# magic-research/vector_quantization

Hardware: AMD Instinct MI355X
Metric: quantized tokens/sec, VQGAN quantizer forward K=16384 D=256 (higher is better)
Workload: dtype f16+f32; 1 GPU; VQGAN K=16384 D=256, 256x256 images -> 16x16 tokens, bf16 latents, VQGANQuantizer.forward of the drop-in nn.Module, eval mode (prepare+argmin+gather+STE+loss); images_per_gpu=2048, parallelism=dp1 (independent shards, no data-path collective)

## Files before the change

vector_quantization_amd/csrc/vqhip.hip:

```cpp
#include "vqhip.h"

#include <hip/hip_runtime.h>
#include <stdio.h>
#include <string.h>

#include "vqhip_kernels.h"
#include "vqhip_fsq_kernels.h"

static thread_local char g_err[256] = "";

static int fail(int code, const char *what, const char *detail = "") {
    snprintf(g_err, sizeof(g_err), "%s%s%s", what, detail[0] ? ": " : "", detail);
    return code;
}

#define VQ_CHECK_LAUNCH(name)                                            \
    do {                                                                 \
        hipError_t err__ = hipGetLastError();                            \
        if (err__ != hipSuccess) return fail(VQHIP_ELAUNCH, name, hipGetErrorString(err__)); \
    } while (0)

#define VQ_HIP(call)                                                     \
    do {                                                                 \
        hipError_t err__ = (call);                                       \
        if (err__ != hipSuccess) return fail(VQHIP_ELAUNCH, #call, hipGetErrorString(err__)); \
    } while (0)

#include <atomic>
#include <mutex>
#include <vector>
static std::atomic<bool> g_prof_on{false};
static std::mutex g_prof_mu;
static std::vector<std::pair<hipEvent_t, hipEvent_t>> g_prof_events;
static size_t g_prof_used = 0;

static long prof_begin(hipStream_t s) {
    if (!g_prof_on.load(std::memory_order_relaxed)) return -1;
    std::lock_guard<std::mutex> lock(g_prof_mu);
    if (g_prof_used == g_prof_events.size()) {
        hipEvent_t a, b;
        if (hipEventCreate(&a) != hipSuccess || hipEventCreate(&b) != hipSuccess) { g_prof_on = false; return -1; }
        g_prof_events.emplace_back(a, b);
    }
    const long slot = (long)g_prof_used++;
    (void)hipEventRecord(g_prof_events[slot].first, s);
    return slot;
}
static void prof_end(long slot, hipStream_t s) {
    if (slot < 0) return;
    std::lock_guard<std::mutex> lock(g_prof_mu);
    if ((size_t)slot < g_prof_events.size()) (void)hipEventRecord(g_prof_events[slot].second, s);
}

#define VQ_MAX_DEVICES 64
typedef std::atomic<size_t> LdsCache[VQ_MAX_DEVICES];
static int ensure_dyn_lds(const void *kern, size_t bytes, LdsCache &set) {
    int dev = 0;
    VQ_HIP(hipGetDevice(&dev));
    const bool cached = dev >= 0 && dev < VQ_MAX_DEVICES;
    if (!cached || bytes > set[dev].load(std::memory_order_acquire)) {
        VQ_HIP(hipFuncSetAttribute(kern, hipFuncAttributeMaxDynamicSharedMemorySize, (int)bytes));
        if (cached) {
            size_t cur = set[dev].load(std::memory_order_relaxed);
            while (cur < bytes && !set[dev].compare_exchange_weak(cur, bytes, std::memory_order_release)) {}
        }
    }
    return VQHIP_OK;
}

#define VQ_NEED(what, have, need)                                                                         \
    do {                                                                                                  \
        const int64_t need__ = (need);                                                                    \
        if ((have) < need__) {                                                                            \
            char msg__[160];                                                                              \
            snprintf(msg__, sizeof(msg__), "%lld bytes given, %lld needed", (long long)(have), (long long)need__); \
            return fail(VQHIP_EINVAL, what, msg__);                                                       \
        }                                                                                                 \
    } while (0)

static inline int waves_grid(int64_t rows, int waves_per_block) {
    return (int)((rows + waves_per_block - 1) / waves_per_block);
}

static std::atomic<int> g_tune_slices{0};
static std::atomic<int> g_tune_force_exact{0};
static std::atomic<int> g_tune_stream{1};
#define VQ_FUSED_DECIDE_MAX_N 16384

template <int NSTEP, int TT, int WAVES, int TPS, int NBUF = 2, bool FILTER = false, bool NOAUX = false, bool GROUPS = false, int XD = 0>
static int launch_coarse_cfg(const char *ximg, int64_t N, const char *frag, int64_t nstages, int nslices, float *rec,
                             int64_t Np, const VqCbStats *cbst, const float *xh2, const float *rho2, int Dp, int metric,
                             const VqDecideOut &dec, int pad_stage, int tpb, hipStream_t s) {
    constexpr int LDS = NBUF * (TPS * NSTEP + VQ_AUX_CHUNKS(TPS)) * VQ_CHUNK_BYTES;
    auto kern = coarse_kernel<NSTEP, TT, WAVES, TPS, NBUF, FILTER, NOAUX, GROUPS, XD>;
    static LdsCache lds_set;
    if (int rc = ensure_dyn_lds((const void *)kern, LDS, lds_set)) return rc;
    const int64_t ntiles = (N + 15) / 16;
    const int64_t ntb = (ntiles + tpb - 1) / tpb;
    const int grid = (int)(ntb * nslices);
    const long slot = prof_begin(s);
    kern<<<grid, WAVES * 64, LDS, s>>>(ximg, N, frag, nstages, nslices, rec, Np, cbst, xh2, rho2, Dp, metric, dec, pad_stage, tpb);
    prof_end(slot, s);
    VQ_CHECK_LAUNCH("coarse_kernel");
    return VQHIP_OK;
}

template <int TT, int WAVES, int TPS, int NBUF, bool NOAUX, int KS>
static int launch_coarse32_cfg(const char *ximg, int64_t N, const char *frag, int64_t nstages, int nslices, float *rec,
                               int64_t Np, const VqCbStats *cbst, const float *xh2, const float *rho2, int Dp, int metric,
                               const int *n_dev, const VqGroupLists &grp, int pad_stage, int tpb, hipStream_t s) {
    constexpr int LDS = NBUF * (TPS * 2 + VQ_AUX_CHUNKS(TPS)) * VQ_CHUNK_BYTES;
    auto kern = coarse32_kernel<TT, WAVES, TPS, NBUF, NOAUX, KS, VQ_GROUP_TILES>;
    static LdsCache lds_set;
    if (int rc = ensure_dyn_lds((const void *)kern, LDS, lds_set)) return rc;
    const int64_t ntiles = (N + 15) / 16;
    const int64_t ntb = (ntiles + tpb - 1) / tpb;
    const long slot = prof_begin(s);
    kern<<<(int)(ntb * nslices), WAVES * 64, LDS, s>>>(ximg, N, frag, nstages, nslices, rec, Np, cbst, xh2, rho2, Dp, metric, n_dev, grp, pad_stage, tpb);
    prof_end(slot, s);
    VQ_CHECK_LAUNCH("coarse32_kernel");
    return VQHIP_OK;
}

template <int NSTEP, int TT, int WAVES, int TPS, int NBUF = 2, int XD = 0>
static int launch_rescan_cfg(const char *ximg, const char *frag, int64_t nstages, const int *rescan_list, const int *counters,
                             const float *thr, int *rescan_cnt, int *cand_list, hipStream_t s, const void *xrows = nullptr) {
    constexpr int LDS = NBUF * (TPS * NSTEP + VQ_AUX_CHUNKS(TPS)) * VQ_CHUNK_BYTES + WAVES * TT * 16 * 4 * (1 + VQ_RESCAN_LOCAL);
    auto kern = rescan_kernel<NSTEP, TT, WAVES, TPS, NBUF, XD>;
    static LdsCache lds_set;
    if (int rc = ensure_dyn_lds((const void *)kern, LDS, lds_set)) return rc;
    kern<<<256, WAVES * 64, LDS, s>>>(ximg, frag, nstages, rescan_list, counters, thr, rescan_cnt, cand_list, xrows);
    VQ_CHECK_LAUNCH("rescan_kernel");
    return VQHIP_OK;
}

#ifndef VQ_W32_MAX_D
#define VQ_W32_MAX_D 32
#endif
#ifndef VQ_NBUF_D32
#define VQ_NBUF_D32 4
#endif
#ifndef VQ_D32_SMALL_TT
#define VQ_D32_SMALL_TT 2
#define VQ_D32_SMALL_W 8
#endif
#ifndef VQ_MIN_SLICES_FILTER
#define VQ_MIN_SLICES_FILTER 1
#endif
static int balanced_tiles_per_block(int64_t N, int full) {
    if (full < 16) return full;
    const int64_t ntiles = (N + 15) / 16;
    int best = full;
    int64_t best_cost = ((ntiles + full - 1) / full + 255) / 256 * full;
    for (int tpb = full - 1; tpb >= full / 2 && tpb >= 8; --tpb) {
        const int64_t cost = ((ntiles + tpb - 1) / tpb + 255) / 256 * tpb;
        if (cost < best_cost) { best_cost = cost; best = tpb; }
    }
    return best;
}

static bool vq_xdirect(int64_t N, int64_t K, int D, int x_dtype, int metric, const int *n_dev) {
    if (D != 256 || n_dev != nullptr || vq_cb_layout(K, D).nstages < 2 || g_tune_slices.load() == 1) return false;
    if (x_dtype != VQHIP_DTYPE_BF16) return false;
    if (metric != VQHIP_METRIC_L2 && metric != VQHIP_METRIC_COS && metric != VQHIP_METRIC_COS_BF16) return false;
    if (N <= VQ_FUSED_DECIDE_MAX_N) return false;
    return !(N <= 4096 || (N <= 256 * 64 && K <= 4096));
}

static int pick_slices(int64_t ntb, int64_t nstages, int min_slices = 2) {
    if (const int forced = g_tune_slices.load(); forced > 0) { int ns = forced; while (ns > 1 && ns > nstages) ns >>= 1; return ns; }
    int64_t want = (256 + ntb - 1) / ntb;
    want = want < min_slices ? min_slices : want;
    int ns = 1;
    while (ns < want && ns < VQ_MAX_SLICES) ns <<= 1;
    while (ns > 1 && ns > nstages) ns >>= 1;
    return ns;
}

struct VqGroupRun { int used, ks, noaux, pad_stage; };
static int launch_coarse(const char *ximg, int64_t N, const VqCbLayout &L, const char *frag, float *rec, int64_t Np,
                         const VqCbStats *cbst, const float *xh2, const float *rho2, int metric, const VqDecideOut &dec,
                         int *nslices_out, int *fused_decide_out, hipStream_t s, VqGroupLists grp = VqGroupLists{nullptr, nullptr, nullptr, nullptr, 0, 1, 0},
                         VqGroupRun *grun = nullptr, bool xd = false) {
    const int nstep = L.nstep;
    const bool small = N <= 256 * 64;
    const bool small16 = N <= 4096 || (N <= 256 * 64 && L.K <= 4096);
    const bool small32 = N < 512 * 512;
    const bool noaux = !VQ_IS_L2(metric);
    const int pad_stage = (L.K % ((int64_t)L.tps * VQ_TILE_CODES)) ? (int)(L.nstages - 1) : -1;
#define VQ_CFG(NS, TT, W, ...)                                                                      \
    {                                                                                               \
        int64_t ntb = (N + (W) * (TT) * 16 - 1) / ((W) * (TT) * 16);                                \
        int ns = pick_slices(ntb, L.nstages, (NS) <= 8 ? VQ_MIN_SLICES_FILTER : 2);                 \
        *nslices_out = ns;                                                                          \
        const int tpb = (ns == 1) ? balanced_tiles_per_block(N, (W) * (TT)) : (W) * (TT);           \
        VqDecideOut dsel = dec;                                                                     \
        if (!(ns == 1 || N <= VQ_FUSED_DECIDE_MAX_N)) dsel.idx = nullptr;                           \
        *fused_decide_out = dsel.idx != nullptr ? 1 : 0;                                            \
        return launch_coarse_cfg<NS, TT, W, __VA_ARGS__>(ximg, N, frag, L.nstages, ns, rec, Np, cbst, xh2, rho2, L.Dp, metric, dsel, pad_stage, tpb, s); \
    }
    switch (nstep) {
        case 2: if ((L.D <= 16 || (L.D <= VQ_W32_MAX_D && noaux)) && N >= VQ_W32_MIN_N && grp.bcnt != nullptr && grun != nullptr) {
                    const int tt = small32 ? 1 : 2;
                    const int full = 8 * tt * 2;
                    const int64_t ntb0 = (N + full * 16 - 1) / (full * 16);
                    int ns = pick_slices(ntb0, L.nstages, VQ_MIN_SLICES_FILTER);
                    ns = ns > VQ_GROUP_MAX_SLICES ? VQ_GROUP_MAX_SLICES : ns;
                    *nslices_out = ns;
                    int tpb = (ns == 1) ? balanced_tiles_per_block(N, full) : full;
                    tpb = (tpb + 1) & ~1;
                    *fused_decide_out = 0;
                    grun->used = 1; grun->ks = L.D <= 16 ? 1 : 2; grun->noaux = noaux ? 1 : 0; grun->pad_stage = pad_stage;
#define VQ_CFG32(TTW, NOAUXV, KSV) return launch_coarse32_cfg<TTW, 8, VQ_TPS_D32, VQ_NBUF_D32, NOAUXV, KSV>(ximg, N, frag, L.nstages, ns, rec, Np, cbst, xh2, rho2, L.Dp, metric, dec.n_dev, grp, pad_stage, tpb, s)
                    if (L.D <= 16) {
                        if (tt == 1) { if (noaux) VQ_CFG32(1, true, 1); else VQ_CFG32(1, false, 1); }
                        else { if (noaux) VQ_CFG32(2, true, 1); else VQ_CFG32(2, false, 1); }
                    } else {
                        if (tt == 1) { if (noaux) VQ_CFG32(1, true, 2); else VQ_CFG32(1, false, 2); }
                        else { if (noaux) VQ_CFG32(2, true, 2); else VQ_CFG32(2, false, 2); }
                    }
#undef VQ_CFG32
                }
                if (N >= VQ_GROUPS_MIN_N) {
                    if (noaux) { if (small32) VQ_CFG(2, VQ_D32_SMALL_TT, VQ_D32_SMALL_W, VQ_TPS_D32, VQ_NBUF_D32, true, true, true) else VQ_CFG(2, 4, 8, VQ_TPS_D32, VQ_NBUF_D32, true, true, true) }
                    if (small32) VQ_CFG(2, VQ_D32_SMALL_TT, VQ_D32_SMALL_W, VQ_TPS_D32, VQ_NBUF_D32, true, false, true) else VQ_CFG(2, 4, 8, VQ_TPS_D32, VQ_NBUF_D32, true, false, true)
                }
                if (noaux) { if (small32) VQ_CFG(2, VQ_D32_SMALL_TT, VQ_D32_SMALL_W, VQ_TPS_D32, VQ_NBUF_D32, true, true) else VQ_CFG(2, 4, 8, VQ_TPS_D32, VQ_NBUF_D32, true, true) }
                if (small32) VQ_CFG(2, VQ_D32_SMALL_TT, VQ_D32_SMALL_W, VQ_TPS_D32, VQ_NBUF_D32, true) else VQ_CFG(2, 4, 8, VQ_TPS_D32, VQ_NBUF_D32, true)
        case 4: if (small) VQ_CFG(4, 2, 8, 4, 4, true) else VQ_CFG(4, 4, 8, 4, 4, true)
        case 8: if (small) VQ_CFG(8, 2, 8, 4, 4, true) else VQ_CFG(8, 4, 8, 4, 4, true)
        case 16: if (xd && !small16) VQ_CFG(16, 4, 8, VQ_TPS16, 4, false, false, false, 1)
                 if (small16) VQ_CFG(16, 2, 8, VQ_TPS16, 4) else VQ_CFG(16, 4, 8, VQ_TPS16, 4)
        case 32: VQ_CFG(32, 2, 8, 2)
        case 48: VQ_CFG(48, 2, 8, 1)
        case 64: {
            auto cost = [&](int tokens, double eff) {
                const int64_t ntb = (N + tokens - 1) / tokens;
                const int ns = pick_slices(ntb, L.nstages, 2);
                return (double)((ntb * ns + 255) / 256) * tokens * ((double)L.nstages / ns) / eff;
            };
            if (cost(192, 1.18) < cost(128, 1.0)) VQ_CFG(64, 3, 4, 1) else VQ_CFG(64, 1, 8, 1)
        }
        default: break;
    }
#undef VQ_CFG
    return fail(VQHIP_EINVAL, "vqhip_argmin: unsupported padded D");
}

static int resident_grid(int per_cu) {
    static std::atomic<int> cus[VQ_MAX_DEVICES];
    int dev = 0, n = 0;
    if (hipGetDevice(&dev) != hipSuccess) return 256 * per_cu;
    if (dev >= 0 && dev < VQ_MAX_DEVICES && (n = cus[dev].load(std::memory_order_relaxed)) > 0) return n * per_cu;
    if (hipDeviceGetAttribute(&n, hipDeviceAttributeMultiprocessorCount, dev) != hipSuccess || n <= 0) n = 256;
    if (dev >= 0 && dev < VQ_MAX_DEVICES) cus[dev].store(n, std::memory_order_relaxed);
    return n * per_cu;
}

template <int MODE>
static int run_exact_tiled(const void *x, int x_dtype, const float *e, const float *en, const float *xn, int64_t N, int64_t K,
                           int D, int metric, u64 *keys, float *dout, hipStream_t s) {
    const int bf = x_dtype == VQHIP_DTYPE_F32 ? 0 : 1;
    const int64_t items = ((N + 127) / 128) * ((K + 255) / 256);
    if (g_tune_stream.load() && D % (bf ? 8 : 4) == 0 && items < (int64_t)1 << 31) {
        static LdsCache ssets[2];
        const int lds = vq_xs_lds_bytes(bf);
        const void *kern = bf ? (const void *)exact_stream_kernel<1, MODE> : (const void *)exact_stream_kernel<0, MODE>;
        if (int rc = ensure_dyn_lds(kern, lds, ssets[bf])) return rc;
        const int cap = resident_grid(2);
        const int grid = (int)(items < cap ? items : cap);
        if (bf) exact_stream_kernel<1, MODE><<<grid, 256, lds, s>>>(x, e, en, xn, N, K, D, metric, keys, dout);
        else exact_stream_kernel<0, MODE><<<grid, 256, lds, s>>>(x, e, en, xn, N, K, D, metric, keys, dout);
        VQ_CHECK_LAUNCH("exact_stream_kernel");
        return VQHIP_OK;
    }
    constexpr int LDS = 2 * 32 * 128 * 4 + 8 * 32 * 4;
    static LdsCache sets[4];
    const void *kerns[4] = {(const void *)exact_tiled_kernel<0, MODE, false>, (const void *)exact_tiled_kernel<1, MODE, false>,
                            (const void *)exact_tiled_kernel<0, MODE, true>, (const void *)exact_tiled_kernel<1, MODE, true>};
    const int v4 = (D % 4 == 0) ? 2 : 0;
    if (int rc = ensure_dyn_lds(kerns[v4 + bf], LDS, sets[v4 + bf])) return rc;
    int grid = (int)(items < 1024 ? items : 1024);
#define VQ_TILED(DT, V4) exact_tiled_kernel<DT, MODE, V4><<<grid, 256, LDS, s>>>(x, e, en, xn, N, K, D, metric, keys, dout)
    if (v4) { if (bf) VQ_TILED(1, true); else VQ_TILED(0, true); }
    else { if (bf) VQ_TILED(1, false); else VQ_TILED(0, false); }
#undef VQ_TILED
    VQ_CHECK_LAUNCH("exact_tiled_kernel");
    return VQHIP_OK;
}

static int exact_few_max(int D) {
    if (D > 512 || D > VQ_FEW_MAX_D) return 0;
    static std::atomic<int> lds_limit{-1};
    int lim = lds_limit.load(std::memory_order_relaxed);
    if (lim < 0) {
        int dev = 0, v = 0;
        if (hipGetDevice(&dev) != hipSuccess || hipDeviceGetAttribute(&v, hipDeviceAttributeMaxSharedMemoryPerBlock, dev) != hipSuccess) v = 65536;
        lim = v;
        lds_limit.store(lim);
    }
    return vq_few_lds_bytes(D) <= lim ? VQ_EXACT_FEW_MAX : 0;
}

static int run_exact_rows(const void *x, int x_dtype, const float *e, const float *en, const float *xn, int64_t N, int64_t K, int D,
                          int metric, const int *row_list, const int *nrows_dev, u64 *keys, int *ticket, int64_t *idx,
                          int32_t *hist, hipStream_t s) {
    const int64_t ncb = (K + 63) / 64;
    const int grid = (int)(ncb < 256 ? 256 : (ncb > 1024 ? 1024 : ncb));
    if (D % 4) return fail(VQHIP_EINVAL, "exact_kernel: D % 4 != 0 (the proposal route has D % 8 == 0)");
    const int few_max = exact_few_max(D);
    const int lds = few_max ? vq_few_lds_bytes(D) : 0;
    static LdsCache sets[2];
    const int bf = x_dtype == VQHIP_DTYPE_F32 ? 0 : 1;
    if (int rc = ensure_dyn_lds(bf ? (const void *)exact_kernel<1> : (const void *)exact_kernel<0>, lds, sets[bf])) return rc;
    if (!bf)
        exact_kernel<0><<<grid, 256, lds, s>>>(x, e, en, xn, N, K, D, metric, row_list, nrows_dev, keys, ticket, idx, hist, few_max);
    else
        exact_kernel<1><<<grid, 256, lds, s>>>(x, e, en, xn, N, K, D, metric, row_list, nrows_dev, keys, ticket, idx, hist, few_max);
    VQ_CHECK_LAUNCH("exact_kernel");
    return VQHIP_OK;
}

template <int MODE>
static int run_segsum(const void *src, int x_dtype, const float *e, const int64_t *idx, const int32_t *order,
                      const int32_t *offsets, int64_t N, int64_t K, int D, const float *g_cb, float *dst, void *ws,
                      hipStream_t s) {
    float *partial = (float *)ws;
    const int64_t nranges = (N + VQ_SEG_RANGE - 1) / VQ_SEG_RANGE;
    int grid = (int)((nranges + 3) / 4); grid = grid < 1 ? 1 : (grid > 4096 ? 4096 : grid);
    if (x_dtype == VQHIP_DTYPE_F32) segsum_rows_kernel<MODE, 0><<<grid, 256, 0, s>>>(src, e, idx, order, offsets, N, (int)K, D, g_cb, dst, partial);
    else segsum_rows_kernel<MODE, 1><<<grid, 256, 0, s>>>(src, e, idx, order, offsets, N, (int)K, D, g_cb, dst, partial);
    VQ_CHECK_LAUNCH("segsum_rows_kernel");
    int fgrid = (int)((K + 3) / 4); fgrid = fgrid > 2048 ? 2048 : fgrid;
    segsum_fixup_kernel<<<fgrid, 256, 0, s>>>(offsets, (int)K, D, partial, dst);
    VQ_CHECK_LAUNCH("segsum_fixup_kernel");
    return VQHIP_OK;
}

template <bool NORMALIZE>
static int launch_row_small(const void *v, int dtype, int64_t R, int D, float eps, float *out, hipStream_t s) {
    const int L = D <= 8 ? 8 : (D <= 16 ? 16 : 32);
    const int grid = waves_grid((R + 64 / L - 1) / (64 / L), 4);
#define VQ_ROW_SMALL(DT, LL) row_small_kernel<DT, LL, NORMALIZE><<<grid, 256, 0, s>>>(v, R, D, eps, out)
    if (dtype == VQHIP_DTYPE_F32) { if (L == 8) VQ_ROW_SMALL(0, 8); else if (L == 16) VQ_ROW_SMALL(0, 16); else VQ_ROW_SMALL(0, 32); }
    else { if (L == 8) VQ_ROW_SMALL(1, 8); else if (L == 16) VQ_ROW_SMALL(1, 16); else VQ_ROW_SMALL(1, 32); }
#undef VQ_ROW_SMALL
    VQ_CHECK_LAUNCH("row_small_kernel");
    return VQHIP_OK;
}

extern "C" {

int vqhip_version(void) { return VQHIP_VERSION; }
const char *vqhip_last_error(void) { return g_err; }

int64_t vqhip_codebook_exact_offset(int64_t K, int D) {
    if (K <= 0 || D <= 0) return -1;
    return vq_cb_layout(K, D).off_eexact;
}

static int launch_vqkd_front(const float *w_in, float *w_mid, int64_t K, const void *x, int x_dtype, float *xn, int64_t N, int D, float eps,
                             float *zero, int64_t nzero, int w_passes, hipStream_t s) {
    if (D <= 32) {
        const int L = D <= 8 ? 8 : (D <= 16 ? 16 : 32), rpb = 4 * (64 / L);
        const int kblocks = (int)((K + rpb - 1) / rpb), xblocks = (int)((N + rpb - 1) / rpb);
#define VQ_FRONT_SMALL(DT, LL) vqkd_front_small_kernel<DT, LL><<<kblocks + xblocks, 256, 0, s>>>(w_in, w_mid, K, x, xn, N, D, eps, kblocks, zero, nzero, w_passes)
        if (x_dtype == VQHIP_DTYPE_F32) { if (L == 8) VQ_FRONT_SMALL(0, 8); else if (L == 16) VQ_FRONT_SMALL(0, 16); else VQ_FRONT_SMALL(0, 32); }
        else { if (L == 8) VQ_FRONT_SMALL(1, 8); else if (L == 16) VQ_FRONT_SMALL(1, 16); else VQ_FRONT_SMALL(1, 32); }
#undef VQ_FRONT_SMALL
    } else {
        const int kblocks = (int)((K + 3) / 4), xblocks = (int)((N + 3) / 4);
        if (x_dtype == VQHIP_DTYPE_F32) vqkd_front_kernel<0><<<kblocks + xblocks, 256, 0, s>>>(w_in, w_mid, K, x, xn, N, D, eps, kblocks, zero, nzero, w_passes);
        else vqkd_front_kernel<1><<<kblocks + xblocks, 256, 0, s>>>(w_in, w_mid, K, x, xn, N, D, eps, kblocks, zero, nzero, w_passes);
    }
    VQ_CHECK_LAUNCH("vqkd_front_kernel");
    return VQHIP_OK;
}

int64_t vqhip_codebook_bytes(int64_t K, int D) {
    if (K <= 0 || D <= 0) return 0;
    return vq_cb_layout(K, D).total;
}

int64_t vqhip_workspace_bytes(int64_t N, int64_t K, int D) {
// ... 1396 lines not shown
```

vector_quantization_amd/csrc/vqhip_proposal_kernels.h:

```cpp
#pragma once
struct Top2 { float v1, v2, v3; uint32_t c1, c2; };
__device__ __forceinline__ float row_margin(const VqCbStats *st, int Dp, int metric, float X2, float R2, float *bf16_part = nullptr);

struct VqDecideOut {
    int64_t *idx; int32_t *hist;
    int *rescan_list, *multi_list, *exact_list, *counters;
    u64 *keys; float *thr_out; int *rescan_cnt;
    int *arrive;
    const int *n_dev;
    const void *xrows; float *xh2_w, *rho2_w, *xn_w;
};
template <bool AGENT>
__device__ __forceinline__ void decide_rows(int64_t n, bool oob, const VqCbStats *st, int Dp, int metric, int nslices,
                                            const float *rec, const float *xh2, const float *rho2, int64_t Np,
                                            const VqDecideOut &o, int *wcount, int *wbase, const float *rece2 = nullptr);

__device__ __forceinline__ void top_insert(Top2 &t, float v, uint32_t c) {
    if (v > t.v1) { t.v3 = fmaxf(t.v3, t.v2); t.v2 = t.v1; t.c2 = t.c1; t.v1 = v; t.c1 = c; }
    else if (v > t.v2) { t.v3 = fmaxf(t.v3, t.v2); t.v2 = v; t.c2 = c; }
    else t.v3 = fmaxf(t.v3, v);
}

__device__ __forceinline__ void top_merge_lane(Top2 &t, int xor_mask) {
    Top2 o;
    o.v1 = __shfl_xor(t.v1, xor_mask, 64); o.v2 = __shfl_xor(t.v2, xor_mask, 64); o.v3 = __shfl_xor(t.v3, xor_mask, 64);
    o.c1 = __shfl_xor(t.c1, xor_mask, 64); o.c2 = __shfl_xor(t.c2, xor_mask, 64);
    if (o.c1 != 0xFFFFFFFFu) top_insert(t, o.v1, o.c1);
    if (o.c2 != 0xFFFFFFFFu) top_insert(t, o.v2, o.c2);
    t.v3 = fmaxf(t.v3, o.v3);
}

__device__ __forceinline__ int tile_row16(int e, int lane) { return 16 * (e >> 2) + 4 * (lane >> 4) + (e & 3); }

#ifndef VQ_D32_PLAIN_OCC
#define VQ_D32_PLAIN_OCC 2
#endif
template <int NSTEP, int TT, int WAVES, int TPS, int NBUF = 2, bool FILTER = false, bool NOAUX = false,
          bool GROUPS = false, int XD = 0>
__global__ __launch_bounds__(WAVES * 64, (FILTER && NSTEP <= 2) ? (GROUPS ? 4 : VQ_D32_PLAIN_OCC) : WAVES / 4) void coarse_kernel(
    const char *__restrict__ ximg, int64_t N, const char *__restrict__ frag, int64_t nstages, int nslices,
    float *__restrict__ rec, int64_t Np, const VqCbStats *__restrict__ cbst, const float *__restrict__ xh2,
    const float *__restrict__ rho2, int Dp, int metric, VqDecideOut dec, int pad_stage, int tpb) {
    extern __shared__ __attribute__((aligned(16))) char lds[];
    static_assert(NSTEP % 2 == 0, "16x16x32 layout: 32-dim k-steps");
    static_assert(!GROUPS || FILTER, "group records are a form of the filtered epilogue");
    constexpr bool GBRANCH = TT >= VQ_GROUP_BRANCH_MIN_TT;
    constexpr bool PIPE = (TPS % 2) == 0;
    constexpr bool PIPE_H = (TPS == 1) && (WAVES <= 4);
    static_assert(!(PIPE_H && (NOAUX || FILTER)), "half-tile ping-pong: plain large-D form only");
    constexpr int NS32 = NSTEP / 2;
    constexpr int NCH = TPS * NSTEP + VQ_AUX_CHUNKS(TPS);
    constexpr int STAGE_BYTES = NCH * VQ_CHUNK_BYTES;
    constexpr int NE = 8;
#ifndef VQ_SCALAR_WAVE
#define VQ_SCALAR_WAVE 1
#endif
    const int lane = threadIdx.x & 63;
    const int wave = (VQ_SCALAR_WAVE && NSTEP > 2) ? __builtin_amdgcn_readfirstlane((int)(threadIdx.x >> 6)) : (int)(threadIdx.x >> 6);
    const int64_t ntt = (N + 31) / 32 * 2;
    if (dec.n_dev != nullptr) {
        const int64_t nd = *dec.n_dev;
        N = nd < N ? nd : N;
        if ((int64_t)(blockIdx.x / nslices) * tpb * 16 >= N) return;
    }
    const bool wave_active = wave * TT < tpb;
    cb_stats_publish(cbst);
    const int sl = blockIdx.x % nslices;
    const int64_t tb = blockIdx.x / nslices;
    const int64_t st0 = (nstages * sl) / nslices, st1 = (nstages * (sl + 1)) / nslices;
  for (bool once = true; once; once = false) {

    half8 xf[TT][NS32];
    if constexpr (XD == 0) {
#pragma unroll
        for (int t = 0; t < TT; ++t) {
            int64_t tt = tb * tpb + wave * TT + t;
            tt = tt < ntt ? tt : ntt - 1;
            const char *src = ximg + tt * (int64_t)(NS32 * VQ_CHUNK_BYTES) + lane * 16;
#pragma unroll
            for (int s = 0; s < NS32; ++s) xf[t][s] = *(const half8 *)(src + s * VQ_CHUNK_BYTES);
        }
    } else {
        static_assert(XD == 1 && !FILTER && !GROUPS && !NOAUX && (NSTEP % 4) == 0, "token side in the prologue: bf16 rows, plain D % 64 == 0 forms");
        const int q4 = lane >> 4, r16 = lane & 15;
        constexpr int Dr = NS32 * 32;
        static_assert(NS32 == 8 && NBUF >= 4 && 2 * STAGE_BYTES >= WAVES * 16 * 528, "row tile: D = 256, staged behind stage 1");
        char *stg = lds + 2 * STAGE_BYTES + wave * (16 * 528);
        const int hr = lane >> 5, c32 = lane & 31;
#pragma unroll
        for (int t = 0; t < TT; ++t) {
            const int64_t tok0 = (tb * tpb + wave * TT + t) * 16;
#pragma unroll
            for (int i = 0; i < 8; ++i) {
                const int64_t tok = tok0 + 2 * i + hr;
                const int64_t trow = tok < N ? tok : N - 1;
                xf[t][i] = *(const half8 *)((const uint16_t *)dec.xrows + trow * Dr + 8 * c32);
            }
        }
        __builtin_amdgcn_sched_barrier(0);
#pragma unroll
        for (int t = 0; t < TT; ++t) {
#pragma unroll
            for (int i = 0; i < 8; ++i) *(half8 *)(stg + (2 * i + hr) * 528 + 16 * c32) = xf[t][i];
#pragma unroll
            for (int s = 0; s < NS32; ++s) xf[t][s] = *(const half8 *)(stg + r16 * 528 + 64 * s + 16 * q4);
        }
#pragma unroll
        for (int t = 0; t < TT; ++t) {
            const int64_t tok = (tb * tpb + wave * TT + t) * 16 + r16;
            [[maybe_unused]] const int64_t trow = tok < N ? tok : N - 1;
            const bool stats = sl == 0;
            float sh[2] = {0.0f, 0.0f}, sr[2] = {0.0f, 0.0f}, pn[2][8];
#pragma unroll
            for (int j = 0; j < 8; ++j) { pn[0][j] = 0.0f; pn[1][j] = 0.0f; }
#pragma unroll
            for (int s = 0; s < NS32; ++s) {
                float v[8];
                half8 f;
                typedef uint32_t u32x4 __attribute__((ext_vector_type(4)));
                typedef _Float16 half2v __attribute__((ext_vector_type(2)));
                typedef float float2v __attribute__((ext_vector_type(2)));
                const u32x4 bits = __builtin_bit_cast(u32x4, xf[t][s]);
#pragma unroll
                for (int j = 0; j < 4; ++j) {
                    const uint32_t lo = bits[j] << 16, hi = bits[j] & 0xFFFF0000u;
                    v[2 * j] = __uint_as_float(lo); v[2 * j + 1] = __uint_as_float(hi);
                    float2v c;
                    c[0] = (lo & 0x7FFFFFFFu) < 0x38800000u ? 0.0f : v[2 * j];
                    c[1] = (hi & 0x7FFFFFFFu) < 0x38800000u ? 0.0f : v[2 * j + 1];
                    const half2v h = __builtin_convertvector(c, half2v);
                    f[2 * j] = h[0]; f[2 * j + 1] = h[1];
                }
                if (stats) {
#pragma unroll
                    for (int j = 0; j < 8; ++j) {
                        const float b = (float)f[j], res = v[j] - b;
                        sh[s & 1] = fmaf(b, b, sh[s & 1]); sr[s & 1] = fmaf(res, res, sr[s & 1]);
                        pn[s & 1][j] = fmaf(v[j], v[j], pn[s & 1][j]);
                    }
                }
                xf[t][s] = f;
            }
            if (!stats) continue;
            float a = 0.0f, b = 0.0f;
#pragma unroll
            for (int g = 0; g < 8; ++g) {
                a += __shfl(sh[g >> 2], (g & 3) * 16 + r16, 64);
                b += __shfl(sr[g >> 2], (g & 3) * 16 + r16, 64);
            }
            float q[8];
#pragma unroll
            for (int j = 0; j < 8; ++j) q[j] = pn[0][j] + pn[1][j];
#pragma unroll
            for (int j = 0; j < 8; ++j) q[j] = q[j] + __shfl_xor(q[j], 32, 64);
#pragma unroll
            for (int j = 0; j < 8; ++j) q[j] = q[j] + __shfl_xor(q[j], 16, 64);
            float a0 = q[0] + q[4], a1 = q[1] + q[5], a2 = q[2] + q[6], a3 = q[3] + q[7];
            a0 = a0 + a2; a1 = a1 + a3;
            a0 = a0 + a1;
            if (sl == 0 && q4 == 0 && tok < N && wave * TT + t < tpb) { dec.xh2_w[tok] = a; dec.rho2_w[tok] = b; dec.xn_w[tok] = a0; }
        }
    }
    if constexpr (PIPE_H) {
#pragma unroll
        for (int t = 0; t < TT; ++t)
#pragma unroll
            for (int s = 0; s < NS32; ++s) {
                if (t >= TT / 2) asm volatile("" : "+a"(xf[t][s]));
                else asm volatile("" : "+v"(xf[t][s]));
            }
    }

    float b1[TT], b2[TT], th[TT], mg[TT];
    uint32_t t1[TT];
#pragma unroll
    for (int t = 0; t < TT; ++t) { b1[t] = -INFINITY; b2[t] = -INFINITY; th[t] = -INFINITY; mg[t] = INFINITY; t1[t] = 0; }
    static_assert(!FILTER || PIPE, "the filtered epilogue is written for the ping-pong form");
    float sc0 = 0.0f, sc1 = 0.0f, sc2 = 0.0f;
    if constexpr (FILTER) {
        const VqCbStats stv = cb_stats_view(cbst);
#pragma unroll
        for (int t = 0; t < TT; ++t) {
            int64_t tokn = (tb * tpb + wave * TT + t) * 16 + (lane & 15);
            tokn = tokn < N ? tokn : N - 1;
            const float m = row_margin(&stv, Dp, metric, xh2[tokn], rho2[tokn]);
            mg[t] = (m > 0.0f) ? m : INFINITY;
        }
    }

    auto issue_stage = [&](int64_t st, int buf) {
        const char *src = frag + st * (int64_t)STAGE_BYTES;
        char *dstb = lds + buf * STAGE_BYTES;
        for (int c = wave; c < NCH; c += WAVES)
            __builtin_amdgcn_global_load_lds(
                (const __attribute__((address_space(1))) void *)(src + c * VQ_CHUNK_BYTES + lane * 16),
                (__attribute__((address_space(3))) void *)(dstb + c * VQ_CHUNK_BYTES), 16, 0, 0);
    };

    constexpr int AHEAD = NBUF >= 3 ? 2 : 1;
#ifndef VQ_LAG_MIN_STAGES
#define VQ_LAG_MIN_STAGES 48
#endif
    const int lag = (NBUF >= 4 && wave >= WAVES / 2 && st1 - st0 >= VQ_LAG_MIN_STAGES) ? 1 : 0;
    if (st0 < st1) issue_stage(st0, 0);
    if (AHEAD >= 2 && st0 + 1 < st1) issue_stage(st0 + 1, 1);
    vq_dma_barrier();

    f32x4 accA[2][TT], accB[2][TT];
#pragma unroll
    for (int c = 0; c < 2; ++c)
#pragma unroll
        for (int t = 0; t < TT; ++t)
#pragma unroll
            for (int q = 0; q < 4; ++q)
                accB[c][t][q] = GROUPS ? -INFINITY : -3.0e38f;
    if constexpr (PIPE_H) {
#pragma unroll
        for (int t = 0; t < TT; ++t) accA[1][t] = f32x4{-3.0e38f, -3.0e38f, -3.0e38f, -3.0e38f};
    }

    for (int64_t it = st0; it < st1 + ((NBUF >= 4 && st1 - st0 >= VQ_LAG_MIN_STAGES) ? 1 : 0); ++it) {
        if (it + AHEAD < st1) issue_stage(it + AHEAD, (int)((it + AHEAD - st0) % NBUF));
        const int64_t st = it - lag;
        if (st < st0 || st >= st1 || !wave_active) { vq_dma_barrier(); continue; }
        const int buf = (int)((st - st0) % NBUF);
        const char *base = lds + buf * STAGE_BYTES;
        const char *aux = base + TPS * NSTEP * VQ_CHUNK_BYTES;
      auto run_stage = [&](auto with_aux_tag) __attribute__((always_inline)) {
        constexpr bool WITH_AUX = decltype(with_aux_tag)::value;
        if constexpr (PIPE_H) {
            constexpr int PFH = VQ_PIPEH_PF;
            constexpr int TOTALH = 4 * TT;
            const uint32_t tile = (uint32_t)st;
#pragma unroll
            for (int c = 0; c < 2; ++c) {
                const f32x4 a4 = *(const f32x4 *)(aux + (16 * c + 4 * (lane >> 4)) * 4);
                uint32_t old[TT];
#pragma unroll
                for (int t = 0; t < TT; ++t) { accA[c][t] = a4; old[t] = __float_as_uint(b1[t]); }
                half8 af[PFH + 1];
#pragma unroll
                for (int i = 0; i < PFH; ++i) af[i] = *(const half8 *)(base + (2 * i + c) * VQ_CHUNK_BYTES + lane * 16);
#pragma unroll
                for (int s = 0; s < NS32; ++s) {
                    if (s + PFH < NS32)
                        af[(s + PFH) % (PFH + 1)] = *(const half8 *)(base + (2 * (s + PFH) + c) * VQ_CHUNK_BYTES + lane * 16);
#pragma unroll
                    for (int t = 0; t < TT; ++t)
                        accA[c][t] = __builtin_amdgcn_mfma_f32_16x16x32_f16(af[s % (PFH + 1)], xf[t][s], accA[c][t], 0, 0, 0);
#pragma unroll
                    for (int id = s * TOTALH / NS32; id < (s + 1) * TOTALH / NS32; ++id) {
                        const int t = id / 4, q = id % 4, e = 4 * (1 - c) + q;
                        float v = __uint_as_float((__float_as_uint(accA[1 - c][t][q]) & 0xFFFFFFF0u) | (uint32_t)e);
                        b2[t] = __builtin_amdgcn_fmed3f(b1[t], b2[t], v);
                        b1[t] = vmax(b1[t], v);
                    }
                    __builtin_amdgcn_sched_barrier(0);
                }
                const uint32_t tgp = tile - (c == 0 ? 1u : 0u);
#pragma unroll
                for (int t = 0; t < TT; ++t) t1[t] = (__float_as_uint(b1[t]) != old[t]) ? tgp : t1[t];
            }
        } else {
#ifndef VQ_PF_TT2
#define VQ_PF_TT2 3
#endif
#ifndef VQ_PF_TT4
#define VQ_PF_TT4 2
#endif
#ifndef VQ_CHUNK_SB
#define VQ_CHUNK_SB 2
#endif
#ifndef VQ_STAGE_PF
#define VQ_STAGE_PF 1
#endif
        constexpr bool CHUNK_SB = NSTEP >= 4 && NSTEP <= 16 && !FILTER && (VQ_CHUNK_SB == 2 || (VQ_CHUNK_SB == 1 && TT <= 2));
        constexpr int PF = NSTEP <= 32 ? (CHUNK_SB ? (TT <= 2 ? VQ_PF_TT2 : VQ_PF_TT4) : 1) : (NSTEP <= 48 ? 2 : 4);
        constexpr bool STAGE_PF = (VQ_STAGE_PF != 0) && CHUNK_SB && TPS >= 2;
        half8 af[PF + 1];
#pragma unroll
        for (int ti = 0; ti < TPS; ++ti) {
            f32x4 (&cur)[2][TT] = (PIPE && (ti & 1)) ? accB : accA;
            f32x4 (&prv)[2][TT] = (PIPE && (ti & 1)) ? accA : accB;
            if constexpr (WITH_AUX) {
#pragma unroll
                for (int c = 0; c < 2; ++c) {
                    f32x4 a4 = *(const f32x4 *)(aux + (ti * 32 + 16 * c + 4 * (lane >> 4)) * 4);
#pragma unroll
                    for (int t = 0; t < TT; ++t) cur[c][t] = a4;
                }
            }
            uint32_t old[TT];
#pragma unroll
            for (int t = 0; t < TT; ++t) old[t] = __float_as_uint(b1[t]);
            constexpr int RING = PF + 1;
            const int g0 = STAGE_PF ? ti * NSTEP : 0;
            if (!STAGE_PF || ti == 0) {
#pragma unroll
                for (int i = 0; i < PF; ++i)
                    if (i < NSTEP) af[i] = *(const half8 *)(base + (ti * NSTEP + i) * VQ_CHUNK_BYTES + lane * 16);
            }
#pragma unroll
            for (int ch = 0; ch < NSTEP; ++ch) {
                if (ch + PF < NSTEP || (STAGE_PF && ti + 1 < TPS))
                    af[(g0 + ch + PF) % RING] = *(const half8 *)(base + (ti * NSTEP + ch + PF) * VQ_CHUNK_BYTES + lane * 16);
#pragma unroll
                for (int t = 0; t < TT; ++t) {
                    if constexpr (!WITH_AUX) {
                        if (ch < 2) {
                            cur[ch & 1][t] = __builtin_amdgcn_mfma_f32_16x16x32_f16(af[(g0 + ch) % RING], xf[t][ch >> 1], f32x4{0.0f, 0.0f, 0.0f, 0.0f}, 0, 0, 0);
                            continue;
                        }
                    }
                    cur[ch & 1][t] = __builtin_amdgcn_mfma_f32_16x16x32_f16(af[(g0 + ch) % RING], xf[t][ch >> 1], cur[ch & 1][t], 0, 0, 0);
                }
                if constexpr (FILTER) {
                    const uint32_t tgp = (uint32_t)(st * TPS + ti) - 1u;
#pragma unroll
                    for (int i = 0; i < (TT + NSTEP - 1) / NSTEP; ++i) {
                        constexpr int EVERY = (NSTEP / TT) > 0 ? NSTEP / TT : 1;
                        const int t = (TT >= NSTEP) ? ch * (TT / NSTEP) + i : ((ch % EVERY == 0) ? ch / EVERY : -1);
                        if (t >= 0 && t < TT) {
                            float after[TT];
#pragma unroll
                            for (int u = 0; u < TT; ++u) after[u] = cur[ch & 1][u][0];
                            tile_max8<TT>(sc0, sc1, sc2, prv[0][t], prv[1][t], after);
                            if constexpr (GROUPS) {
                                if (!GBRANCH || __any(!(sc0 < th[t]))) {
                                    const float nb = vmax(b1[t], sc0);
                                    b2[t] = __builtin_amdgcn_fmed3f(b1[t], b2[t], sc0);
                                    t1[t] = (__float_as_uint(nb) != __float_as_uint(b1[t])) ? tgp : t1[t];
                                    b1[t] = nb;
                                }
                            } else if (__any(!(sc0 < th[t]))) {
                                const uint32_t was = __float_as_uint(b1[t]);
#pragma unroll
                                for (int e = 0; e < NE; ++e) {
                                    float v = __uint_as_float((__float_as_uint(prv[e >> 2][t][e & 3]) & 0xFFFFFFF0u) | (uint32_t)e);
                                    b2[t] = __builtin_amdgcn_fmed3f(b1[t], b2[t], v);
                                    b1[t] = vmax(b1[t], v);
                                }
                                t1[t] = (__float_as_uint(b1[t]) != was) ? tgp : t1[t];
                            }
                        }
                    }
                }
                constexpr int TOTAL = NE * TT;
                constexpr bool RETIRE = PIPE && !FILTER;
#pragma unroll
                for (int i = 0; RETIRE && i < (TOTAL + NSTEP - 1) / NSTEP; ++i) {
                    constexpr int EVERY = (NSTEP / TOTAL) > 0 ? NSTEP / TOTAL : 1;
                    const int id = (TOTAL >= NSTEP) ? ch * (TOTAL / NSTEP) + i : ((ch % EVERY == 0) ? ch / EVERY : -1);
                    if (id >= 0 && id < TOTAL) {
                        const int t = id / NE, e = id % NE;
                        float v = __uint_as_float((__float_as_uint(prv[e >> 2][t][e & 3]) & 0xFFFFFFF0u) | (uint32_t)e);
                        b2[t] = __builtin_amdgcn_fmed3f(b1[t], b2[t], v);
                        b1[t] = vmax(b1[t], v);
                    }
                }
                if constexpr (CHUNK_SB) __builtin_amdgcn_sched_barrier(0);
            }
            if constexpr (!PIPE && !PIPE_H) {
#pragma unroll
                for (int t = 0; t < TT; ++t)
#pragma unroll
                    for (int e = 0; e < NE; ++e) {
                        float v = __uint_as_float((__float_as_uint(cur[e >> 2][t][e & 3]) & 0xFFFFFFF0u) | (uint32_t)e);
                        b2[t] = __builtin_amdgcn_fmed3f(b1[t], b2[t], v);
                        b1[t] = vmax(b1[t], v);
                    }
            }
            if constexpr (!FILTER) {
                const uint32_t tgp = (uint32_t)(st * TPS + ti) - (PIPE ? 1u : 0u);
#pragma unroll
                for (int t = 0; t < TT; ++t)
                    t1[t] = (__float_as_uint(b1[t]) != old[t]) ? tgp : t1[t];
            }
        }
        }
      };
        if constexpr (NOAUX) {
            if (st == (int64_t)pad_stage) run_stage(std::true_type{}); else run_stage(std::false_type{});
        } else {
            run_stage(std::true_type{});
        }
        if constexpr (FILTER && (!GROUPS || GBRANCH)) {
#pragma unroll
            for (int t = 0; t < TT; ++t) th[t] = quad_rows_max(b1[t]) - mg[t];
        }
        vq_dma_barrier();
    }
    if (PIPE_H && st1 > st0) {
#pragma unroll
        for (int t = 0; t < TT; ++t) {
            const uint32_t old = __float_as_uint(b1[t]);
#pragma unroll
            for (int q = 0; q < 4; ++q) {
                float v = __uint_as_float((__float_as_uint(accA[1][t][q]) & 0xFFFFFFF0u) | (uint32_t)(4 + q));
                b2[t] = __builtin_amdgcn_fmed3f(b1[t], b2[t], v);
                b1[t] = vmax(b1[t], v);
            }
            t1[t] = (__float_as_uint(b1[t]) != old) ? (uint32_t)(st1 * TPS - 1) : t1[t];
        }
    }
    if (PIPE && st1 > st0) {
#pragma unroll
        for (int t = 0; t < TT; ++t) {
            const uint32_t old = __float_as_uint(b1[t]);
            if constexpr (GROUPS) {
                float g = accB[0][t][0];
#pragma unroll
                for (int e = 1; e < NE; ++e) g = __builtin_amdgcn_fmed3f(g, accB[e >> 2][t][e & 3], INFINITY);
                b2[t] = __builtin_amdgcn_fmed3f(b1[t], b2[t], g);
                b1[t] = vmax(b1[t], g);
            } else {
#pragma unroll
                for (int e = 0; e < NE; ++e) {
                    float v = __uint_as_float((__float_as_uint(accB[e >> 2][t][e & 3]) & 0xFFFFFFF0u) | (uint32_t)e);
                    b2[t] = __builtin_amdgcn_fmed3f(b1[t], b2[t], v);
                    b1[t] = vmax(b1[t], v);
                }
            }
            t1[t] = (__float_as_uint(b1[t]) != old) ? (uint32_t)(st1 * TPS - 1) : t1[t];
        }
    }

    bool ident[TT];
#pragma unroll
    for (int t = 0; t < TT; ++t) ident[t] = true;
    if constexpr (GROUPS) {
        auto bound_up = [](float v) {
            const uint32_t b = __float_as_uint(v);
            return __uint_as_float((b & 0x80000000u) ? (b & 0xFFFFFFF0u) : (b | 0xFu));
        };
        constexpr int RB = NSTEP <= 2 ? VQ_REPLAY_BATCH : (NSTEP <= 4 ? 2 : 1);
#pragma unroll
        for (int t = 0; t < TT; ++t) {
            const float top = quad_rows_max(b1[t]);
            const int64_t tokn = (tb * tpb + wave * TT + t) * 16 + (lane & 15);
            const bool need = (mg[t] < INFINITY) && (b1[t] > -INFINITY) && !(b1[t] < top - mg[t]) && tokn < N && wave * TT + t < tpb &&
                              t1[t] >= (uint32_t)(st0 * TPS) && t1[t] < (uint32_t)(st1 * TPS);
            float e1 = -INFINITY, e2 = -INFINITY;
            u64 todo = __ballot(need);
            while (todo) {
                uint32_t T[RB];
                u64 rest = todo;
#pragma unroll
                for (int i = 0; i < RB; ++i) {
                    const int l = rest ? (__ffsll((unsigned long long)rest) - 1) : (__ffsll((unsigned long long)todo) - 1);
                    T[i] = (uint32_t)__builtin_amdgcn_readlane((int)t1[t], l);
                    rest &= rest - 1;
                }
                half8 a[RB][NSTEP];
                f32x4 acc[RB][2];
#pragma unroll
                for (int i = 0; i < RB; ++i) {
                    const int64_t rst = T[i] / TPS;
                    const int rti = (int)(T[i] % TPS);
                    const char *sb = frag + rst * (int64_t)STAGE_BYTES;
#pragma unroll
                    for (int ch = 0; ch < NSTEP; ++ch)
                        a[i][ch] = *(const half8 *)(sb + (rti * NSTEP + ch) * VQ_CHUNK_BYTES + lane * 16);
#pragma unroll
                    for (int c = 0; c < 2; ++c) {
                        if (NOAUX && rst != (int64_t)pad_stage) acc[i][c] = f32x4{0.0f, 0.0f, 0.0f, 0.0f};
                        else acc[i][c] = *(const f32x4 *)(sb + TPS * NSTEP * VQ_CHUNK_BYTES + (rti * 32 + 16 * c + 4 * (lane >> 4)) * 4);
                    }
                }
                u64 done = 0;
#pragma unroll
                for (int i = 0; i < RB; ++i) {
#pragma unroll
                    for (int ch = 0; ch < NSTEP; ++ch)
                        acc[i][ch & 1] = __builtin_amdgcn_mfma_f32_16x16x32_f16(a[i][ch], xf[t][ch >> 1], acc[i][ch & 1], 0, 0, 0);
                    float w1 = -INFINITY, w2 = -INFINITY;
#pragma unroll
                    for (int e = 0; e < NE; ++e) {
                        float v = __uint_as_float((__float_as_uint(acc[i][e >> 2][e & 3]) & 0xFFFFFFF0u) | (uint32_t)e);
                        w2 = __builtin_amdgcn_fmed3f(w1, w2, v);
                        w1 = vmax(w1, v);
                    }
                    const bool mine = need && t1[t] == T[i];
                    e1 = mine ? w1 : e1; e2 = mine ? w2 : e2;
                    done |= __ballot(mine);
                }
                todo &= ~done;
            }
            const float other = bound_up(b2[t]);
            if (need) { b1[t] = e1; b2[t] = fmaxf(other, e2); }
            else { b2[t] = fmaxf(other, bound_up(b1[t])); }
            ident[t] = need;
        }
    }

#pragma unroll
    for (int t = 0; t < TT; ++t) {
        Top2 r; r.v1 = r.v2 = r.v3 = -INFINITY; r.c1 = r.c2 = 0xFFFFFFFFu;
        {
            uint32_t bits = __float_as_uint(b1[t]);
            uint32_t code = t1[t] * 32u + (uint32_t)tile_row16((int)(bits & 7u), lane);
            if (ident[t] && b1[t] > -INFINITY) top_insert(r, b1[t], code);
            r.v3 = fmaxf(r.v3, b2[t]);
        }
        top_merge_lane(r, 16);
        top_merge_lane(r, 32);
        const int64_t tokn = (tb * tpb + wave * TT + t) * 16 + (lane & 15);
        if (lane < 16 && tokn < N && wave * TT + t < tpb) {
            float *rp = rec + (int64_t)sl * VQ_REC_FIELDS * Np + tokn;
            if (dec.idx != nullptr && nslices > 1) {
                __hip_atomic_store(rp, r.v1, __ATOMIC_RELAXED, __HIP_MEMORY_SCOPE_AGENT);
                __hip_atomic_store(rp + Np, __uint_as_float(r.c1), __ATOMIC_RELAXED, __HIP_MEMORY_SCOPE_AGENT);
                __hip_atomic_store(rp + 2 * Np, r.v2, __ATOMIC_RELAXED, __HIP_MEMORY_SCOPE_AGENT);
                __hip_atomic_store(rp + 3 * Np, __uint_as_float(r.c2), __ATOMIC_RELAXED, __HIP_MEMORY_SCOPE_AGENT);
                __hip_atomic_store(rp + 4 * Np, r.v3, __ATOMIC_RELAXED, __HIP_MEMORY_SCOPE_AGENT);
            } else {
                rp[0] = r.v1; rp[Np] = __uint_as_float(r.c1); rp[2 * Np] = r.v2;
                rp[3 * Np] = __uint_as_float(r.c2); rp[4 * Np] = r.v3;
            }
        }
    }

    if (dec.idx != nullptr) {
        int *flags = (int *)lds;
        asm volatile("s_waitcnt vmcnt(0)" ::: "memory");
        __syncthreads();
        if (threadIdx.x == 0) {
            int last = 1;
            if (nslices > 1) {
                last = (atomicAdd(&dec.arrive[tb], 1) == nslices - 1) ? 1 : 0;
            }
            flags[0] = last;
        }
        __syncthreads();
        const bool last = flags[0] != 0;
        __syncthreads();
        if (last) {
            int *wcount = (int *)lds, *wbase = wcount + 3 * 16;
            int64_t n = tb * (int64_t)(tpb * 16) + threadIdx.x;
            const bool oob = (int)threadIdx.x >= tpb * 16 || n >= N;
            if (n >= N) n = N - 1;
            decide_rows<true>(n, oob, cbst, Dp, metric, nslices, rec, xh2, rho2, Np, dec, wcount, wbase);
        }
    }
  }
}
```

Measured before the change: 148.6 million tokens/s.

## Add segment form: one block scans all codebook stages, emitting per-segment records

Adds an XD==2 variant of the coarse kernel where each block handles every codebook stage for its token tile instead of splitting stages across slice blocks. At each segment boundary the block flushes a top-2 record into that segment's slot and resets its running state, so the fused decide step still sees nslices records. It drops the cross-block arrival atomics and the duplicated token-tile loads across slices, at the cost of a smaller grid. It is chosen when the tile-block count fills whole waves of 256 blocks.

```diff
diff --git a/vector_quantization_amd/csrc/vqhip.hip b/vector_quantization_amd/csrc/vqhip.hip
--- a/vector_quantization_amd/csrc/vqhip.hip
+++ b/vector_quantization_amd/csrc/vqhip.hip
@@ -97,7 +97,7 @@
     if (int rc = ensure_dyn_lds((const void *)kern, LDS, lds_set)) return rc;
     const int64_t ntiles = (N + 15) / 16;
     const int64_t ntb = (ntiles + tpb - 1) / tpb;
-    const int grid = (int)(ntb * nslices);
+    const int grid = (int)(XD == 2 ? ntb : ntb * nslices);
     const long slot = prof_begin(s);
     kern<<<grid, WAVES * 64, LDS, s>>>(ximg, N, frag, nstages, nslices, rec, Np, cbst, xh2, rho2, Dp, metric, dec, pad_stage, tpb);
     prof_end(slot, s);
@@ -175,6 +175,11 @@
     while (ns < want && ns < VQ_MAX_SLICES) ns <<= 1;
     while (ns > 1 && ns > nstages) ns >>= 1;
     return ns;
+}
+
+static bool vq_segment_form(int64_t ntb) {
+    if (g_tune_slices.load() > 0) return true;
+    return ntb >= 256 && 2 * ((ntb + 255) / 256) <= (2 * ntb + 255) / 256;
 }
 
 struct VqGroupRun { int used, ks, noaux, pad_stage; };
@@ -229,7 +234,16 @@
                 if (small32) VQ_CFG(2, VQ_D32_SMALL_TT, VQ_D32_SMALL_W, VQ_TPS_D32, VQ_NBUF_D32, true) else VQ_CFG(2, 4, 8, VQ_TPS_D32, VQ_NBUF_D32, true)
         case 4: if (small) VQ_CFG(4, 2, 8, 4, 4, true) else VQ_CFG(4, 4, 8, 4, 4, true)
         case 8: if (small) VQ_CFG(8, 2, 8, 4, 4, true) else VQ_CFG(8, 4, 8, 4, 4, true)
-        case 16: if (xd && !small16) VQ_CFG(16, 4, 8, VQ_TPS16, 4, false, false, false, 1)
+        case 16: if (xd && !small16) {
+                     const int64_t ntb = (N + 511) / 512;
+                     if (vq_segment_form(ntb)) {
+                         const int nseg = pick_slices(ntb, L.nstages, 2);
+                         *nslices_out = nseg;
+                         *fused_decide_out = 1;
+                         return launch_coarse_cfg<16, 4, 8, VQ_TPS16, 4, false, false, false, 2>(ximg, N, frag, L.nstages, nseg, rec, Np, cbst, xh2, rho2, L.Dp, metric, dec, pad_stage, 32, s);
+                     }
+                     VQ_CFG(16, 4, 8, VQ_TPS16, 4, false, false, false, 1)
+                 }
                  if (small16) VQ_CFG(16, 2, 8, VQ_TPS16, 4) else VQ_CFG(16, 4, 8, VQ_TPS16, 4)
         case 32: VQ_CFG(32, 2, 8, 2)
         case 48: VQ_CFG(48, 2, 8, 1)
diff --git a/vector_quantization_amd/csrc/vqhip_proposal_kernels.h b/vector_quantization_amd/csrc/vqhip_proposal_kernels.h
--- a/vector_quantization_amd/csrc/vqhip_proposal_kernels.h
+++ b/vector_quantization_amd/csrc/vqhip_proposal_kernels.h
@@ -65,9 +65,10 @@
     }
     const bool wave_active = wave * TT < tpb;
     cb_stats_publish(cbst);
-    const int sl = blockIdx.x % nslices;
-    const int64_t tb = blockIdx.x / nslices;
-    const int64_t st0 = (nstages * sl) / nslices, st1 = (nstages * (sl + 1)) / nslices;
+    constexpr bool SEG = XD == 2;
+    const int sl = SEG ? 0 : blockIdx.x % nslices;
+    const int64_t tb = SEG ? blockIdx.x : blockIdx.x / nslices;
+    const int64_t st0 = SEG ? 0 : (nstages * sl) / nslices, st1 = SEG ? nstages : (nstages * (sl + 1)) / nslices;
   for (bool once = true; once; once = false) {
 
     half8 xf[TT][NS32];
@@ -81,7 +82,7 @@
             for (int s = 0; s < NS32; ++s) xf[t][s] = *(const half8 *)(src + s * VQ_CHUNK_BYTES);
         }
     } else {
-        static_assert(XD == 1 && !FILTER && !GROUPS && !NOAUX && (NSTEP % 4) == 0, "token side in the prologue: bf16 rows, plain D % 64 == 0 forms");
+        static_assert((XD == 1 || XD == 2) && !FILTER && !GROUPS && !NOAUX && (NSTEP % 4) == 0, "token side in the prologue: bf16 rows, plain D % 64 == 0 forms");
         const int q4 = lane >> 4, r16 = lane & 15;
         constexpr int Dr = NS32 * 32;
         static_assert(NS32 == 8 && NBUF >= 4 && 2 * STAGE_BYTES >= WAVES * 16 * 528, "row tile: D = 256, staged behind stage 1");
@@ -219,6 +220,9 @@
         for (int t = 0; t < TT; ++t) accA[1][t] = f32x4{-3.0e38f, -3.0e38f, -3.0e38f, -3.0e38f};
     }
 
+    static_assert(!SEG || (PIPE && !GROUPS && !PIPE_H && !FILTER), "segment form: the plain ping-pong epilogue");
+    [[maybe_unused]] int seg = 0;
+    [[maybe_unused]] int64_t seg_end = SEG ? nstages / nslices : st1;
     for (int64_t it = st0; it < st1 + ((NBUF >= 4 && st1 - st0 >= VQ_LAG_MIN_STAGES) ? 1 : 0); ++it) {
         if (it + AHEAD < st1) issue_stage(it + AHEAD, (int)((it + AHEAD - st0) % NBUF));
         const int64_t st = it - lag;
@@ -388,6 +392,38 @@
 #pragma unroll
             for (int t = 0; t < TT; ++t) th[t] = quad_rows_max(b1[t]) - mg[t];
         }
+        if constexpr (SEG) {
+            if (st + 1 == seg_end && st + 1 < st1) {
+#pragma unroll
+                for (int t = 0; t < TT; ++t) {
+                    const uint32_t old = __float_as_uint(b1[t]);
+#pragma unroll
+                    for (int e = 0; e < NE; ++e) {
+                        float v = __uint_as_float((__float_as_uint(accB[e >> 2][t][e & 3]) & 0xFFFFFFF0u) | (uint32_t)e);
+                        b2[t] = __builtin_amdgcn_fmed3f(b1[t], b2[t], v);
+                        b1[t] = vmax(b1[t], v);
+                    }
+                    t1[t] = (__float_as_uint(b1[t]) != old) ? (uint32_t)(seg_end * TPS - 1) : t1[t];
+                    Top2 r; r.v1 = r.v2 = r.v3 = -INFINITY; r.c1 = r.c2 = 0xFFFFFFFFu;
+                    const uint32_t code = t1[t] * 32u + (uint32_t)tile_row16((int)(__float_as_uint(b1[t]) & 7u), lane);
+                    if (b1[t] > -INFINITY) top_insert(r, b1[t], code);
+                    r.v3 = fmaxf(r.v3, b2[t]);
+                    top_merge_lane(r, 16);
+                    top_merge_lane(r, 32);
+                    const int64_t tokn = (tb * tpb + wave * TT + t) * 16 + (lane & 15);
+                    if (lane < 16 && tokn < N && wave * TT + t < tpb) {
+                        float *rp = rec + (int64_t)seg * VQ_REC_FIELDS * Np + tokn;
+                        rp[0] = r.v1; rp[Np] = __uint_as_float(r.c1); rp[2 * Np] = r.v2;
+                        rp[3 * Np] = __uint_as_float(r.c2); rp[4 * Np] = r.v3;
+                    }
+                    b1[t] = -INFINITY; b2[t] = -INFINITY; t1[t] = 0;
+#pragma unroll
+                    for (int c = 0; c < 2; ++c) accB[c][t] = f32x4{-3.0e38f, -3.0e38f, -3.0e38f, -3.0e38f};
+                }
+                ++seg;
+                seg_end = (nstages * (seg + 1)) / nslices;
+            }
+        }
         vq_dma_barrier();
     }
     if (PIPE_H && st1 > st0) {
@@ -506,8 +542,8 @@
         top_merge_lane(r, 32);
         const int64_t tokn = (tb * tpb + wave * TT + t) * 16 + (lane & 15);
         if (lane < 16 && tokn < N && wave * TT + t < tpb) {
-            float *rp = rec + (int64_t)sl * VQ_REC_FIELDS * Np + tokn;
-            if (dec.idx != nullptr && nslices > 1) {
+            float *rp = rec + (int64_t)(SEG ? seg : sl) * VQ_REC_FIELDS * Np + tokn;
+            if (!SEG && dec.idx != nullptr && nslices > 1) {
                 __hip_atomic_store(rp, r.v1, __ATOMIC_RELAXED, __HIP_MEMORY_SCOPE_AGENT);
                 __hip_atomic_store(rp + Np, __uint_as_float(r.c1), __ATOMIC_RELAXED, __HIP_MEMORY_SCOPE_AGENT);
                 __hip_atomic_store(rp + 2 * Np, r.v2, __ATOMIC_RELAXED, __HIP_MEMORY_SCOPE_AGENT);
@@ -526,7 +562,7 @@
         __syncthreads();
         if (threadIdx.x == 0) {
             int last = 1;
-            if (nslices > 1) {
+            if (!SEG && nslices > 1) {
                 last = (atomicAdd(&dec.arrive[tb], 1) == nslices - 1) ? 1 : 0;
             }
             flags[0] = last;
@@ -539,7 +575,8 @@
             int64_t n = tb * (int64_t)(tpb * 16) + threadIdx.x;
             const bool oob = (int)threadIdx.x >= tpb * 16 || n >= N;
             if (n >= N) n = N - 1;
-            decide_rows<true>(n, oob, cbst, Dp, metric, nslices, rec, xh2, rho2, Np, dec, wcount, wbase);
+            if constexpr (SEG) decide_rows<true>(n, oob, cbst, Dp, metric, nslices, rec, dec.xh2_w, dec.rho2_w, Np, dec, wcount, wbase);
+            else decide_rows<true>(n, oob, cbst, Dp, metric, nslices, rec, xh2, rho2, Np, dec, wcount, wbase);
         }
     }
   }
```

After: 147.2 million tokens/s. No clear change (-1.0%).
